# shichaoy/cube_slam

Hardware: NVIDIA H100
Metric: scored cuboid proposals/s (higher is better)
Workload: dtype f64

## Files before the change

### cube_slam_b200/csrc/cs_lsd.cu

```cuda
#include <cuda_runtime.h>
#include <float.h>
#include <math.h>
#include <stdint.h>

#include <algorithm>
#include <cmath>
#include <cstring>
#include <vector>

#include "cs_internal.h"
#include "cs_nfa.cuh"
#include "cs_tma.cuh"

#define LSD_PI 3.1415926535897932384626433832795
#define LSD_NOTDEF (-1024.0)
#define LSD_DEG2RAD (LSD_PI / 180)
#define LSD_3_2_PI ((3 * LSD_PI) / 2)
#define LSD_2PI (2 * LSD_PI)
#define LSD_LN10 2.30258509299404568402
#define LSD_NBINS 1024
#define LSD_CHUNK_ROWS 8
#define LSD_SCALE 0.8

#define LSD_CAND_CAP 2048
#define LSD_SEQ_SCAP 2048
#define LSD_SEQ_SMEM (LSD_SEQ_SCAP * 4 + 96 * 8)
#define LSD_HDR 8

namespace {

struct LsdGeom {
    int64_t img_off;
    int32_t w, h, stride, channels;
    int32_t W, H;
    int32_t min_reg_size, tile0;
    double LOG_NT;
    int64_t px_off;
    int64_t bit_off;
    int64_t arena_off;
    int32_t tiles_x, pad_;
};

__constant__ double c_gauss7[7] = {0x1.763496d347532p-13, 0x1.f1e23259cfdc1p-7, 0x1.bfd7fac1bd5a8p-3, 0x1.10562a79786afp-1,
                                   0x1.bfd7fac1bd5a8p-3, 0x1.f1e23259cfdc1p-7, 0x1.763496d347532p-13};

__device__ __forceinline__ int reflect101(int p, int n)
{
    if (n == 1) return 0;
    while (p < 0 || p >= n) p = (p < 0) ? -p : 2 * n - 2 - p;
    return p;
}

__device__ __forceinline__ float fast_atan2(float y, float x)
{
    const float p1 = 0.9997878412794807f * (float)(180 / LSD_PI);
    const float p3 = -0.3258083974640975f * (float)(180 / LSD_PI);
    const float p5 = 0.1555786518463281f * (float)(180 / LSD_PI);
    const float p7 = -0.04432655554792128f * (float)(180 / LSD_PI);
    const float ax = fabsf(x), ay = fabsf(y);
    float a, c, c2;
    if (ax >= ay) {
        c = ay / (ax + (float)DBL_EPSILON);
        c2 = c * c;
        a = (((p7 * c2 + p5) * c2 + p3) * c2 + p1) * c;
    } else {
        c = ax / (ay + (float)DBL_EPSILON);
        c2 = c * c;
        a = 90.f - (((p7 * c2 + p5) * c2 + p3) * c2 + p1) * c;
    }
    if (x < 0) a = 180.f - a;
    if (y < 0) a = 360.f - a;
    return a;
}

__device__ __forceinline__ void lsd_resize_col(int dx, int sw, double inv_scale, int &sx, float &fx, bool &single)
{
    fx = (float)((dx + 0.5) * inv_scale - 0.5);
    sx = (int)floorf(fx);
    fx -= sx;
    single = false;
    if (sx < 0) {
        fx = 0;
        sx = 0;
    }
    if (sx + 1 >= sw) {
        single = true;
        if (sx >= sw - 1) {
            fx = 0;
            sx = sw - 1;
        }
    }
}
__device__ __forceinline__ void lsd_resize_row(int dy, int sh, double inv_scale, int &y0, int &y1, float &fy)
{
    fy = (float)((dy + 0.5) * inv_scale - 0.5);
    const int sy = (int)floorf(fy);
    fy -= sy;
    y0 = (sy >= 0) ? (sy < sh ? sy : sh - 1) : 0;
    y1 = (sy + 1 >= 0) ? (sy + 1 < sh ? sy + 1 : sh - 1) : 0;
}

#define LSF_TW 32
#define LSF_TH 16
#define LSF_BW 44
#define LSF_BH 24
#define LSF_GW (LSF_BW + 6)
#define LSF_GH (LSF_BH + 6)
#define LSF_BOXW 176
#define LSF_P_BYTES (LSF_GH * LSF_BW * 8)
static_assert(LSF_GH * LSF_BOXW <= LSF_P_BYTES && (LSF_TH + 1) * (LSF_TW + 1) * 8 <= LSF_P_BYTES, "front-end shared-memory aliasing");
template <bool kTma, bool kDebug, bool kMixed>
__global__ void __launch_bounds__(256) k_lsd_front(const __grid_constant__ CUtensorMap tmap, const uint8_t *__restrict__ img, int w, int h, int stride,
                                                   int channels, int W, int H, double inv_scale, double threshold, double *__restrict__ modgrad,
                                                   float *__restrict__ angf, uint4 *__restrict__ pix, uint32_t *__restrict__ defb,
                                                   double *__restrict__ scaled, int32_t *__restrict__ err_flag, const LsdGeom *__restrict__ geom,
                                                   int n_geom)
{
    static_assert(!(kMixed && (kTma || kDebug)), "a mixed batch has no tensor map and no debug form");
    __shared__ __align__(128) unsigned char s_p[LSF_P_BYTES];
    __shared__ double s_b[LSF_BH][LSF_BW];
    __shared__ uint8_t s_g[LSF_GH][LSF_GW];
    __shared__ __align__(8) unsigned long long s_bar;
    double(*s_h)[LSF_BW] = reinterpret_cast<double(*)[LSF_BW]>(s_p);
    double(*s_sc)[LSF_TW + 1] = reinterpret_cast<double(*)[LSF_TW + 1]>(s_p);
    int f = blockIdx.z, X0 = blockIdx.x * LSF_TW, Y0 = blockIdx.y * LSF_TH;
// ... 85 lines not shown
        double s = c_gauss7[3] * s_h[r + 3][c];
#pragma unroll
        for (int k = 1; k <= 3; k++) s += c_gauss7[3 + k] * (s_h[r + 3 + k][c] + s_h[r + 3 - k][c]);
        s_b[r][c] = s;
    }
    __syncthreads();
    for (int i = tid; i < (LSF_TH + 1) * (LSF_TW + 1); i += 256) {
        const int r = i / (LSF_TW + 1), c = i - r * (LSF_TW + 1);
        if (Y0 + r > yl || X0 + c > xl) continue;
        int sx, y0, y1;
        float fx, fy;
        bool single;
        lsd_resize_col(X0 + c, w, inv_scale, sx, fx, single);
        lsd_resize_row(Y0 + r, h, inv_scale, y0, y1, fy);
        const double *S0 = s_b[y0 - by0], *S1 = s_b[y1 - by0];
        const int cx = sx - bx0;
        const float a0 = 1.f - fx, a1 = fx, b0 = 1.f - fy, b1 = fy;
        double r0, r1;
        if (!single) {
            r0 = S0[cx] * a0 + S0[cx + 1] * a1;
            r1 = S1[cx] * a0 + S1[cx + 1] * a1;
        } else {
            r0 = S0[cx] * 1.0;
            r1 = S1[cx] * 1.0;
        }
        s_sc[r][c] = r0 * b0 + r1 * b1;
    }
    __syncthreads();
    const int WW = (W + 31) >> 5;
    for (int i = tid; i < LSF_TH * LSF_TW; i += 256) {
        const int r = i / LSF_TW, c = i - r * LSF_TW;
        const int x = X0 + c, y = Y0 + r;
        float deg = -1.f;
        if (x < W && y < H) {
            const size_t p = kMixed ? (size_t)y * W + x : ((size_t)f * H + y) * W + x;
            double norm = 0;
            if (x < W - 1 && y < H - 1) {
                const double DA = s_sc[r + 1][c + 1] - s_sc[r][c];
                const double BC = s_sc[r][c + 1] - s_sc[r + 1][c];
                const double gx = DA + BC, gy = DA - BC;
                norm = sqrt((gx * gx + gy * gy) / 4);
                if (!kDebug && !(norm <= threshold)) deg = fast_atan2((float)gx, (float)(-gy));
            }
            if (kDebug) {
                scaled[p] = s_sc[r][c];
                modgrad[p] = norm;
            } else {
                angf[p] = deg;
                uint4 rec = make_uint4(__float_as_uint(deg), 0u, 0u, 0u);
                if (deg >= 0.f) {
                    modgrad[p] = norm;
                    const double ang = (double)deg * LSD_DEG2RAD;
                    const double af = (double)(float)ang;
                    rec.y = __float_as_uint((float)cos(af));
                    rec.z = __float_as_uint((float)sin(af));
                }
                pix[p] = rec;
            }
        }
        if (!kDebug) {
            const uint32_t bits = __ballot_sync(0xffffffffu, deg >= 0.f);
            if (c == 0 && y < H) defb[(kMixed ? (size_t)y : (size_t)f * H + y) * WW + (X0 >> 5)] = bits;
        }
    }
}

__device__ unsigned long long g_lsd_prof[16];
#define LSD_PROF_T0() const long long prof_t0__ = kProf ? clock64() : 0ll
#define LSD_PROF_ADD(slot)                                                                         \
    do {                                                                                           \
        if (kProf && (threadIdx.x & 31) == 0) atomicAdd(&g_lsd_prof[slot], (unsigned long long)(clock64() - prof_t0__)); \
    } while (0)
#define LSD_PROF_COUNT(slot, v)                                                    \
    do {                                                                           \
        if (kProf && (threadIdx.x & 31) == 0) atomicAdd(&g_lsd_prof[slot], (unsigned long long)(v)); \
    } while (0)
#define LSD_PROF_RECT_SIZE(n) LSD_PROF_COUNT(15, (n) <= 32 ? 1ull : (n) <= 64 ? 1ull << 21 : 1ull << 42)

extern __shared__ __align__(8) int s_seq[];
__device__ __forceinline__ double *lsd_stage() { return reinterpret_cast<double *>(s_seq + LSD_SEQ_SCAP); }

struct LsdFrame {
    int W, H;
    uint4 *pix;
    const float *angf;
    const double *modgrad;
    double LOG_NT;
    uint32_t *ubits;
    int WW;
    __device__ __forceinline__ uint32_t *used_at(int y, int x, uint32_t &bit) const
    {
        bit = 1u << (x & 31);
        return ubits + y * WW + (x >> 5);
    }
    struct LsdSpan *span;
    const double *lgam;
    unsigned long long wmagic;
    __device__ __forceinline__ int row_of(int addr) const { return (int)(((unsigned long long)(unsigned)addr * wmagic) >> 40); }
};

struct LsdReg {
    int *g;
    int cap;
    __device__ __forceinline__ int get(int i) const { return i < LSD_SEQ_SCAP ? s_seq[i] : g[i]; }
    __device__ __forceinline__ void put(int i, int v) const
    {
        if (i < LSD_SEQ_SCAP)
            s_seq[i] = v;
        else
            g[i] = v;
    }
};

__device__ __forceinline__ void lsd_prefetch_l2(const void *p) { asm volatile("prefetch.global.L2 [%0];" ::"l"(p)); }

struct LsdRect {
    double x1, y1, x2, y2, width, x, y, theta, dx, dy, prec, p;
};

__device__ __forceinline__ double lsd_dist_sq(double x1, double y1, double x2, double y2) { return (x2 - x1) * (x2 - x1) + (y2 - y1) * (y2 - y1); }
__device__ __forceinline__ double lsd_dist(double x1, double y1, double x2, double y2) { return sqrt(lsd_dist_sq(x1, y1, x2, y2)); }
__device__ __forceinline__ double lsd_angle_diff_signed(double a, double b)
{
    double diff = a - b;
    while (diff <= -LSD_PI) diff += LSD_2PI;
    while (diff > LSD_PI) diff -= LSD_2PI;
    return diff;
}
__device__ __forceinline__ bool lsd_double_equal(double a, double b)
{
    if (a == b) return true;
    const double abs_diff = fabs(a - b);
    const double aa = fabs(a), bb = fabs(b);
    double abs_max = (aa > bb) ? aa : bb;
    if (abs_max < DBL_MIN) abs_max = DBL_MIN;
    return (abs_diff / abs_max) <= (100.0 * DBL_EPSILON);
}
__device__ __forceinline__ bool lsd_aligned_deg(float deg, double theta, double prec)
{
    if (deg < 0.f) return false;
    {
        float nf = fabsf((float)theta - deg * 0.017453292f);
        if (nf > 4.712389f) nf = fabsf(nf - 6.2831855f);
        const float pf = (float)prec;
        if (nf < pf - 2e-4f) return true;
        if (nf > pf + 2e-4f) return false;
    }
    const double a = (double)deg * LSD_DEG2RAD;
    double n_theta = theta - a;
    if (n_theta < 0) n_theta = -n_theta;
    if (n_theta > LSD_3_2_PI) {
        n_theta -= LSD_2PI;
        if (n_theta < 0) n_theta = -n_theta;
    }
    return n_theta <= prec;
}

__device__ __noinline__ double lsd_log_gamma(double x)
{
    if (x > 15.0) return 0.918938533204673 + (x - 0.5) * log(x) - x + 0.5 * x * log(x * sinh(1 / x) + 1 / (810.0 * pow(x, 6.0)));
    const double q[7] = {75122.6331530, 80916.6278952, 36308.2951477, 8687.24529705, 1168.92649479, 83.8676043424, 2.50662827511};
    double a = (x + 0.5) * log(x + 5.5) - (x + 5.5);
    double b = 0;
    for (int n = 0; n < 7; ++n) {
        a -= log(x + (double)n);
        b += q[n] * pow(x, (double)n);
    }
    return a + log(b);
}

__device__ __noinline__ double lsd_nfa(int n, int k, double p, double LOG_NT)
{
    if (n == 0 || k == 0) return -LOG_NT;
    if (n == k) return -LOG_NT - (double)n * log10(p);
    const double p_term = p / (1 - p);
    const double log1term = ((double)n + 1) - lsd_log_gamma((double)k + 1) - lsd_log_gamma((double)(n - k) + 1) + (double)k * log(p) + (double)(n - k) * log(1.0 - p);
    double term = exp(log1term);
    if (lsd_double_equal(term, 0)) {
        if (k > n * p) return -log1term / LSD_LN10 - LOG_NT;
        return -LOG_NT;
    }
    double bin_tail = term;
    const double tolerance = 0.1;
    for (int i = k + 1; i <= n; ++i) {
        const double bin_term = (double)(n - i + 1) / (double)i;
        const double mult_term = bin_term * p_term;
        term *= mult_term;
        bin_tail += term;
        if (bin_term < 1) {
            const double err = term * ((1 - pow(mult_term, (double)(n - i + 1))) / (1 - mult_term) - 1);
            if (err < tolerance * fabs(-log10(bin_tail) - LOG_NT) * bin_tail) break;
        }
    }
    return -log10(bin_tail) - LOG_NT;
}

__device__ void lsd_region_grow(const LsdFrame &F, const LsdReg &R, int base, int s_addr, int &reg_size, double &reg_angle, double prec)
{
    const unsigned FULL = 0xffffffffu;
    const int lane = threadIdx.x & 31;
    float reg_deg = F.angf[s_addr];
    reg_angle = (double)reg_deg * LSD_DEG2RAD;
    float sumdx = (float)cos(reg_angle);
    float sumdy = (float)sin(reg_angle);
    __syncwarp();
    if (lane == 0) {
        const int sy = F.row_of(s_addr);
        uint32_t bit;
        uint32_t *w = F.used_at(sy, s_addr - sy * F.W, bit);
        atomicOr(w, bit);
        R.put(base, s_addr);
    }
    reg_size = 1;
    __syncwarp();
    const int grp = lane / 9, kk = lane - grp * 9;
    const int ky = kk / 3 - 1, kx = kk - (kk / 3) * 3 - 1;
    const float precf = (float)prec;
    const unsigned lt_mask = (1u << lane) - 1u;
    for (int i = 0; i < reg_size;) {
        const int navail = min(3, reg_size - i);
        bool cand = false;
        int c_addr = -1;
        float deg = -1.f, csx = 0.f, csy = 0.f;
        if (grp < navail) {
            const int pa = R.get(base + i + grp);
            const int py = F.row_of(pa), px = pa - py * F.W;
            const int yy = py + ky, xx = px + kx;
            if (yy >= 0 && yy < F.H && xx >= 0 && xx < F.W) {
                c_addr = yy * F.W + xx;
                uint32_t ubit;
                const uint32_t *uw_p = F.used_at(yy, xx, ubit);
                const uint4 r = __ldg(F.pix + c_addr);
                const uint32_t uw = __ldcg(uw_p);
                deg = __uint_as_float(r.x);
                if (deg >= 0.f && !(uw & ubit)) {
                    cand = true;
                    csx = __uint_as_float(r.y);
                    csy = __uint_as_float(r.z);
                }
            }
        }
        unsigned maybe = __ballot_sync(FULL, cand);
        if (maybe) {
            float nf = fabsf(reg_deg * 0.017453292f - deg * 0.017453292f);
            if (nf > 4.712389f) nf = fabsf(nf - 6.2831855f);
            const float inv_l = rsqrtf(sumdx * sumdx + sumdy * sumdy) * 1.001f;
            const float per_add = (precf + 0.201f) * inv_l;
            unsigned sure = 0u;
            float D = (float)__popc(maybe) * per_add + 0.0022f;
            if (D <= 0.2f && precf + D < 1.5f) {
                const unsigned m1 = __ballot_sync(FULL, cand && nf < precf + D);
                D = (float)__popc(m1) * per_add + 0.0022f;
                sure = __ballot_sync(FULL, cand && nf < precf - D);
                maybe = __ballot_sync(FULL, cand && nf < precf + D);
            }
            unsigned accepted = 0u;
            bool stale = false;
            while (maybe) {
                const int fl = __ffs(maybe) - 1;
                maybe &= ~(1u << fl);
                if (!((sure >> fl) & 1u)) {
                    if (stale) {
                        reg_deg = fast_atan2(sumdy, sumdx);
                        stale = false;
                    }
                    const bool ok = lsd_aligned_deg(deg, (double)reg_deg * LSD_DEG2RAD, prec);
                    if (!((__ballot_sync(FULL, ok) >> fl) & 1u)) continue;
                }
                const int addrf = __shfl_sync(FULL, c_addr, fl);
                sumdx += __shfl_sync(FULL, csx, fl);
                sumdy += __shfl_sync(FULL, csy, fl);
                stale = true;
                accepted |= 1u << fl;
                maybe &= ~__ballot_sync(FULL, c_addr == addrf);
            }
            if (accepted) {
                if ((accepted >> lane) & 1u) {
                    R.put(base + reg_size + __popc(accepted & lt_mask), c_addr);
                    const int cy = F.row_of(c_addr);
                    uint32_t ubit;
                    uint32_t *uw_p = F.used_at(cy, c_addr - cy * F.W, ubit);
                    atomicOr(uw_p, ubit);
                    const uint4 *q = F.pix + c_addr - 1;
                    if (c_addr >= F.W + 1) lsd_prefetch_l2(q - F.W);
                    lsd_prefetch_l2(q);
                    if (c_addr + F.W + 1 < F.W * F.H) lsd_prefetch_l2(q + F.W);
                }
                reg_size += __popc(accepted);
                if (stale) reg_deg = fast_atan2(sumdy, sumdx);
                __syncwarp();
            }
        }
        i += navail;
    }
    reg_angle = (double)reg_deg * LSD_DEG2RAD;
}

__device__ void lsd_region2rect(const LsdFrame &F, const LsdReg &R, int base, int reg_size, double reg_angle, double prec, double p, LsdRect &rec)
{
    const int lane = threadIdx.x & 31;
    double *st = lsd_stage();
    double x = 0, y = 0, sum = 0;
    for (int i0 = 0; i0 < reg_size; i0 += 32) {
        const int n = min(32, reg_size - i0);
        __syncwarp();
        if (lane < n) {
            const int addr = R.get(base + i0 + lane);
            const double weight = F.modgrad[addr];
            const int ry = F.row_of(addr), rx = addr - ry * F.W;
            st[lane] = (double)rx * weight;
            st[32 + lane] = (double)ry * weight;
            st[64 + lane] = weight;
        }
        __syncwarp();
        for (int j = 0; j < n; j++) {
            x += st[j];
            y += st[32 + j];
            sum += st[64 + j];
        }
    }
    x /= sum;
    y /= sum;
    double Ixx = 0.0, Iyy = 0.0, Ixy = 0.0;
    for (int i0 = 0; i0 < reg_size; i0 += 32) {
        const int n = min(32, reg_size - i0);
        __syncwarp();
        if (lane < n) {
            const int addr = R.get(base + i0 + lane);
            const double weight = F.modgrad[addr];
            const int ry = F.row_of(addr), rx = addr - ry * F.W;
            const double ddx = (double)rx - x, ddy = (double)ry - y;
            st[lane] = ddy * ddy * weight;
            st[32 + lane] = ddx * ddx * weight;
            st[64 + lane] = ddx * ddy * weight;
        }
        __syncwarp();
        for (int j = 0; j < n; j++) {
            Ixx += st[j];
            Iyy += st[32 + j];
            Ixy -= st[64 + j];
        }
    }
    const double lambda = 0.5 * (Ixx + Iyy - sqrt((Ixx - Iyy) * (Ixx - Iyy) + 4.0 * Ixy * Ixy));
    double theta = (fabs(Ixx) > fabs(Iyy)) ? (double)fast_atan2((float)(lambda - Ixx), (float)Ixy) : (double)fast_atan2((float)Ixy, (float)(lambda - Iyy));
    theta *= LSD_DEG2RAD;
    if (fabs(lsd_angle_diff_signed(theta, reg_angle)) > prec) theta += LSD_PI;
    const double dx = cos(theta), dy = sin(theta);
    double l_min = 0, l_max = 0, w_min = 0, w_max = 0;
    for (int i = lane; i < reg_size; i += 32) {
        const int addr = R.get(base + i);
        const int ry = F.row_of(addr), rx = addr - ry * F.W;
        const double regdx = (double)rx - x, regdy = (double)ry - y;
        const double l = regdx * dx + regdy * dy;
        const double w = -regdx * dy + regdy * dx;
        l_max = fmax(l_max, l);
        l_min = fmin(l_min, l);
        w_max = fmax(w_max, w);
        w_min = fmin(w_min, w);
    }
#pragma unroll
    for (int o = 16; o > 0; o >>= 1) {
        l_max = fmax(l_max, __shfl_xor_sync(0xffffffffu, l_max, o));
        l_min = fmin(l_min, __shfl_xor_sync(0xffffffffu, l_min, o));
        w_max = fmax(w_max, __shfl_xor_sync(0xffffffffu, w_max, o));
        w_min = fmin(w_min, __shfl_xor_sync(0xffffffffu, w_min, o));
    }
    rec.x1 = x + l_min * dx;
    rec.y1 = y + l_min * dy;
    rec.x2 = x + l_max * dx;
    rec.y2 = y + l_max * dy;
    rec.width = w_max - w_min;
    rec.x = x;
    rec.y = y;
    rec.theta = theta;
    rec.dx = dx;
    rec.dy = dy;
    rec.prec = prec;
    rec.p = p;
    if (rec.width < 1.0) rec.width = 1.0;
}

__device__ __noinline__ void lsd_region2rect_cold(const LsdFrame &F, const LsdReg &R, int base, int reg_size, double reg_angle, double prec, double p, LsdRect &rec);

template <bool kProf>
__device__ __noinline__ int lsd_reduce_region_radius(const LsdFrame &F, const LsdReg &R, int base, int &reg_size, double reg_angle, double prec, double p,
                                        LsdRect &rec, double density, double density_th)
{
    const unsigned FULL = 0xffffffffu;
    const int lane = threadIdx.x & 31;
    const unsigned lt_mask = (1u << lane) - 1u, gt_mask = ~((2u << lane) - 1u);
    int *st = reinterpret_cast<int *>(lsd_stage());
    const int a0 = R.get(base);
    const double xc = (double)(a0 - F.row_of(a0) * F.W), yc = (double)F.row_of(a0);
    const double radSq1 = lsd_dist_sq(xc, yc, rec.x1, rec.y1), radSq2 = lsd_dist_sq(xc, yc, rec.x2, rec.y2);
    double radSq = radSq1 > radSq2 ? radSq1 : radSq2;
    auto outside = [&](int addr) {
        const int ay = F.row_of(addr), ax = addr - ay * F.W;
        return lsd_dist_sq(xc, yc, (double)ax, (double)ay) > radSq;
    };
    while (density < density_th) {
        radSq *= 0.75 * 0.75;
        const int rs = reg_size;
        int K = 0;
        for (int i0 = 0; i0 < rs; i0 += 32) {
            bool out = false;
            if (i0 + lane < rs) {
                const int addr = R.get(base + i0 + lane);
                out = outside(addr);
                if (out) {
                    const int ay = F.row_of(addr);
                    uint32_t bit;
                    uint32_t *w = F.used_at(ay, addr - ay * F.W, bit);
                    atomicAnd(w, ~bit);
                }
            }
            K += __popc(__ballot_sync(FULL, i0 + lane < rs && !out));
        }
        int hc = -32, dc = (((rs - 1) >> 5) + 1) << 5, dval = 0;
        unsigned hm = 0u, dm = 0u;
        for (;;) {
            while (hm == 0u && hc + 32 < K) {
                hc += 32;
                hm = __ballot_sync(FULL, hc + lane < K && outside(R.get(base + hc + lane)));
            }
            if (hm == 0u) break;
            while (dm == 0u) {
                dc -= 32;
                const int i = dc + lane;
                dval = i < rs ? R.get(base + i) : 0;
                dm = __ballot_sync(FULL, i >= K && i < rs && !outside(dval));
            }
            const int t = min(__popc(hm), __popc(dm));
            const bool give = ((dm >> lane) & 1u) && __popc(dm & gt_mask) < t;
            const bool take = ((hm >> lane) & 1u) && __popc(hm & lt_mask) < t;
            __syncwarp();
            if (give) st[__popc(dm & gt_mask)] = dval;
            __syncwarp();
            if (take) R.put(base + hc + lane, st[__popc(hm & lt_mask)]);
            hm &= ~__ballot_sync(FULL, take);
            dm &= ~__ballot_sync(FULL, give);
        }
        reg_size = K;
        __syncwarp();
        LSD_PROF_COUNT(14, 1);
        if (reg_size < 2) return 3;
        LSD_PROF_RECT_SIZE(reg_size);
        lsd_region2rect_cold(F, R, base, reg_size, reg_angle, prec, p, rec);
        density = (double)reg_size / (lsd_dist(rec.x1, rec.y1, rec.x2, rec.y2) * rec.width);
    }
    return 0;
}

struct LsdSpan {
    int mx, ly, ry, y0, y1;
    int fl, sl, fr, sr;
};

__device__ void lsd_span_setup(const LsdFrame &F, const LsdRect &rec, LsdSpan &P)
{
    const double half_width = rec.width / 2.0;
    const double dyhw = rec.dy * half_width, dxhw = rec.dx * half_width;
    int ox[4], oy[4];
    ox[0] = (int)(rec.x1 - dyhw);
    oy[0] = (int)(rec.y1 + dxhw);
    ox[1] = (int)(rec.x2 - dyhw);
    oy[1] = (int)(rec.y2 + dxhw);
    ox[2] = (int)(rec.x2 + dyhw);
    oy[2] = (int)(rec.y2 - dxhw);
    ox[3] = (int)(rec.x1 + dyhw);
    oy[3] = (int)(rec.y1 - dxhw);
#pragma unroll
    for (int i = 1; i < 4; i++) {
        const int vx = ox[i], vy = oy[i];
        int j = i - 1;
        while (j >= 0 && ((vx == ox[j]) ? (vy < oy[j]) : (vx < ox[j]))) {
            ox[j + 1] = ox[j];
            oy[j + 1] = oy[j];
            j--;
        }
        ox[j + 1] = vx;
        oy[j + 1] = vy;
    }
    int imin = 0, imax = 0;
    for (int i = 1; i < 4; ++i) {
        if (oy[imin] > oy[i]) imin = i;
        if (oy[imax] < oy[i]) imax = i;
    }
    unsigned taken = 1u << imin;
    int ileft = -1;
    for (int i = 0; i < 4; ++i)
        if (!((taken >> i) & 1u)) {
            if (ileft < 0)
                ileft = i;
            else if (ox[ileft] > ox[i])
                ileft = i;
        }
    taken |= 1u << ileft;
    int iright = -1;
    for (int i = 0; i < 4; ++i)
        if (!((taken >> i) & 1u)) {
            if (iright < 0)
                iright = i;
            else if (ox[iright] < ox[i])
// ... 10 lines not shown
        }
    const int mx = ox[imin], my = oy[imin], lx = ox[ileft], ly = oy[ileft], rx = ox[iright], ry = oy[iright], tx = ox[itail];
    P.mx = mx;
    P.ly = ly;
    P.ry = ry;
    P.fl = (my != ly) ? (mx - lx) / (my - ly) : 0;
    P.sl = (ly != tx) ? (lx - tx) / (ly - tx) : 0;
    P.fr = (my != ry) ? (mx - rx) / (my - ry) : 0;
    P.sr = (ry != tx) ? (rx - tx) / (ry - tx) : 0;
    P.y0 = max(my, 0);
    P.y1 = min(oy[imax], F.H - 1);
}

__device__ __forceinline__ void lsd_span_row(const LsdSpan &P, int y, int W, int &lo, int &hi)
{
    const long long n_l2 = (long long)max(0, y - max(P.ly, P.y0)), n_l1 = (long long)(y - P.y0) - n_l2;
    const long long n_r2 = (long long)max(0, y - max(P.ry, P.y0)), n_r1 = (long long)(y - P.y0) - n_r2;
    const long long left_x = (long long)P.mx + n_l1 * (long long)P.fl + n_l2 * (long long)P.sl;
    const long long right_x = (long long)P.mx + n_r1 * (long long)P.fr + n_r2 * (long long)P.sr;
    lo = (int)(left_x > 0 ? left_x : 0);
    hi = (int)(right_x < (long long)(W - 1) ? right_x : (long long)(W - 1));
}

__device__ void lsd_rect_count(const LsdFrame &F, const LsdRect &rec, int &total_pts, int &alg_pts)
{
    const int lane = threadIdx.x & 31;
    LsdSpan P;
    lsd_span_setup(F, rec, P);
    int tot = 0, alg = 0;
    const int n_rows = P.y1 - P.y0 + 1;
    int G = 1;
    while (G < 32 && n_rows * G * 2 <= 32) G <<= 1;
    const int rows_per_step = 32 / G, sub = lane & (G - 1), rsel = lane / G;
    for (int yb = P.y0; yb <= P.y1; yb += rows_per_step) {
        const int y = yb + rsel;
        if (y > P.y1) continue;
        int lo, hi;
        lsd_span_row(P, y, F.W, lo, hi);
        if (hi >= lo) {
            if (sub == 0) tot += hi - lo + 1;
            const float *row = F.angf + (size_t)y * F.W;
            for (int x = lo + sub; x <= hi; x += G) alg += lsd_aligned_deg(row[x], rec.theta, rec.prec) ? 1 : 0;
        }
    }
#pragma unroll
    for (int o = 16; o > 0; o >>= 1) {
        tot += __shfl_xor_sync(0xffffffffu, tot, o);
        alg += __shfl_xor_sync(0xffffffffu, alg, o);
    }
    total_pts = tot;
    alg_pts = alg;
}

__device__ void lsd_rect_count_multi(const LsdFrame &F, const LsdRect *r, int n, bool same_geom, int *tot, int *alg)
{
    const unsigned FULL = 0xffffffffu;
    const int lane = threadIdx.x & 31;
    LsdSpan *sp = F.span;
    const int n_geom = same_geom ? 1 : n;
    __syncwarp();
    if (lane < n_geom) lsd_span_setup(F, r[lane], sp[lane]);
    __syncwarp();
    int y_min = sp[0].y0, y_max = sp[0].y1;
    for (int t = 1; t < n_geom; t++) {
        y_min = min(y_min, sp[t].y0);
        y_max = max(y_max, sp[t].y1);
    }
    const double theta = r[0].theta;
    const float thetaf = (float)theta;
    float pf[5];
#pragma unroll
    for (int t = 0; t < 5; t++) pf[t] = (float)r[t < n ? t : 0].prec;
    int c_tot[5] = {0, 0, 0, 0, 0}, c_alg[5] = {0, 0, 0, 0, 0};
    const int n_rows = y_max - y_min + 1;
    int G = 1;
    while (G < 32 && n_rows * G * 2 <= 32) G <<= 1;
    const int rows_per_step = 32 / G, sub = lane & (G - 1), rsel = lane / G;
    for (int yb = y_min; yb <= y_max; yb += rows_per_step) {
        const int y = yb + rsel;
        if (y > y_max) continue;
        int lo[5], hi[5];
        int x_lo = 0x7fffffff, x_hi = -1;
#pragma unroll
        for (int t = 0; t < 5; t++) {
            lo[t] = 1;
            hi[t] = 0;
            if (t < n_geom && y >= sp[t].y0 && y <= sp[t].y1) {
                lsd_span_row(sp[t], y, F.W, lo[t], hi[t]);
                if (hi[t] >= lo[t]) {
                    x_lo = min(x_lo, lo[t]);
                    x_hi = max(x_hi, hi[t]);
                    if (sub == 0) c_tot[t] += hi[t] - lo[t] + 1;
                }
            }
        }
        if (x_hi < 0) continue;
        const float *row = F.angf + (size_t)y * F.W;
        for (int x = x_lo + sub; x <= x_hi; x += G) {
            const float deg = row[x];
            if (deg < 0.f) continue;
            float nf = fabsf(thetaf - deg * 0.017453292f);
            if (nf > 4.712389f) nf = fabsf(nf - 6.2831855f);
            if (same_geom) {
#pragma unroll
                for (int t = 0; t < 5; t++)
                    if (t < n) {
                        bool a = nf < pf[t] - 2e-4f;
                        if (!a && !(nf > pf[t] + 2e-4f)) a = lsd_aligned_deg(deg, theta, r[t].prec);
                        c_alg[t] += a ? 1 : 0;
                    }
            } else {
                bool a = nf < pf[0] - 2e-4f;
                if (!a && !(nf > pf[0] + 2e-4f)) a = lsd_aligned_deg(deg, theta, r[0].prec);
                if (a) {
#pragma unroll
                    for (int t = 0; t < 5; t++) c_alg[t] += (x >= lo[t] && x <= hi[t]) ? 1 : 0;
                }
            }
        }
    }
    if (same_geom) {
#pragma unroll
        for (int t = 1; t < 5; t++) c_tot[t] = c_tot[0];
    }
#pragma unroll
    for (int t = 0; t < 5; t++) {
#pragma unroll
        for (int o = 16; o > 0; o >>= 1) {
            c_tot[t] += __shfl_xor_sync(FULL, c_tot[t], o);
            c_alg[t] += __shfl_xor_sync(FULL, c_alg[t], o);
        }
        if (t < n) {
            tot[t] = c_tot[t];
            alg[t] = c_alg[t];
        }
    }
}

__device__ __noinline__ void lsd_region2rect_cold(const LsdFrame &F, const LsdReg &R, int base, int reg_size, double reg_angle, double prec, double p, LsdRect &rec)
{
    lsd_region2rect(F, R, base, reg_size, reg_angle, prec, p, rec);
}

template <bool kProf>
__device__ void lsd_grow_candidate(const LsdFrame &F, const LsdReg &R, int s_addr, int min_reg_size, double prec, double p, int &n_all,
                                  int &has_rect, LsdRect &rec)
{
    const double DENSITY_TH = 0.7;
    const int lane = threadIdx.x & 31;
    int base = 0, reg_size = 0, seed = s_addr;
    double reg_angle = 0, tau = prec;
    has_rect = 0;
    n_all = 0;
    for (int pass = 0; pass < 2; pass++) {
        {
            LSD_PROF_T0();
            lsd_region_grow(F, R, base, seed, reg_size, reg_angle, tau);
            LSD_PROF_ADD(pass == 0 ? 0 : 2);
        }
        if (kProf && pass == 0 && lane == 0) {
            atomicAdd(&g_lsd_prof[5], 1ull);
            atomicAdd(&g_lsd_prof[7], (unsigned long long)reg_size);
        }
        n_all = base + reg_size;
        if (reg_size < (pass == 0 ? min_reg_size : 2)) return;
        if (pass == 0) LSD_PROF_COUNT(12, 1);
        LSD_PROF_RECT_SIZE(reg_size);
        {
            LSD_PROF_T0();
            lsd_region2rect(F, R, base, reg_size, reg_angle, prec, p, rec);
            LSD_PROF_ADD(1);
        }
        double density;
        {
            LSD_PROF_T0();
            density = (double)reg_size / (lsd_dist(rec.x1, rec.y1, rec.x2, rec.y2) * rec.width);
            has_rect = density >= DENSITY_TH;
            LSD_PROF_ADD(10);
        }
        if (has_rect) return;
        if (pass == 1) {
            LSD_PROF_T0();
            if (lsd_reduce_region_radius<kProf>(F, R, base, reg_size, reg_angle, prec, p, rec, density, DENSITY_TH) == 0) has_rect = 1;
            LSD_PROF_ADD(11);
            return;
        }
        LSD_PROF_COUNT(13, 1);
        LSD_PROF_T0();
        const int a0 = R.get(base);
        const double xc = (double)(a0 - F.row_of(a0) * F.W), yc = (double)F.row_of(a0);
        const double ang_c = (double)F.angf[a0] * LSD_DEG2RAD;
        double sum = 0, s_sum = 0;
        int n = 0;
        for (int i0 = 0; i0 < reg_size; i0 += 32) {
            const int m = min(32, reg_size - i0);
            bool near = false;
            __syncwarp();
            if (lane < m) {
                const int addr = R.get(base + i0 + lane);
                const int ry = F.row_of(addr), rx = addr - ry * F.W;
                if (lsd_dist(xc, yc, (double)rx, (double)ry) < rec.width) {
                    near = true;
                    const double ang_d = lsd_angle_diff_signed((double)F.angf[addr] * LSD_DEG2RAD, ang_c);
                    lsd_stage()[lane] = ang_d;
                    lsd_stage()[32 + lane] = ang_d * ang_d;
                }
            }
            __syncwarp();
            unsigned todo = __ballot_sync(0xffffffffu, near);
            n += __popc(todo);
            while (todo) {
                const int j = __ffs(todo) - 1;
                todo &= todo - 1;
                sum += lsd_stage()[j];
                s_sum += lsd_stage()[32 + j];
            }
        }
        for (int i = lane; i < reg_size; i += 32) {
            const int addr = R.get(base + i);
            const int ay = F.row_of(addr);
            uint32_t bit;
            uint32_t *w = F.used_at(ay, addr - ay * F.W, bit);
            atomicAnd(w, ~bit);
        }
        __syncwarp();
        const double mean_angle = sum / (double)n;
        tau = 2.0 * sqrt((s_sum - 2.0 * mean_angle * sum) / (double)n + mean_angle * mean_angle);
        seed = a0;
        base += reg_size;
        LSD_PROF_ADD(2);
    }
}

__device__ __forceinline__ bool lsd_keyline_filter(const float *raw, int img_w, int img_h, float line_length_thres, float *o)
{
    const float pre_boundary_thre = 10;
    float e[4] = {raw[0], raw[1], raw[2], raw[3]};
    if (e[0] < 0) e[0] = 0;
    if (e[0] >= img_w) e[0] = (float)img_w - 1.0f;
    if (e[2] < 0) e[2] = 0;
    if (e[2] >= img_w) e[2] = (float)img_w - 1.0f;
    if (e[1] < 0) e[1] = 0;
    if (e[1] >= img_h) e[1] = (float)img_h - 1.0f;
    if (e[3] < 0) e[3] = 0;
    if (e[3] >= img_h) e[3] = (float)img_h - 1.0f;
    const float sx = e[0], sy = e[1], ex = e[2], ey = e[3];
    if (((sx < pre_boundary_thre) && (ex < pre_boundary_thre)) || ((sx > img_w - pre_boundary_thre) && (ex > img_w - pre_boundary_thre)) ||
        ((sy < pre_boundary_thre) && (ey < pre_boundary_thre)) || ((sy > img_h - pre_boundary_thre) && (ey > img_h - pre_boundary_thre)))
        return false;
    const double ddx = (double)(e[0] - e[2]), ddy = (double)(e[1] - e[3]);
    const float line_length = (float)sqrt(ddx * ddx + ddy * ddy);
    if (!(line_length > line_length_thres)) return false;
    o[0] = sx;
    o[1] = sy;
// ... 9 lines not shown
    const double *modgrad;
    int32_t *arena;
    int arena_cap;
    double LOG_NT;
    int min_reg_size;
    double prec, p, scale;
    float line_length_thres;
    float *raw;
    int32_t *n_raw;
    float *out;
    int32_t *n_out;
    int cap;
    LsdRect *cand;
    int32_t *n_cand;
    int cand_cap;
    int32_t *cand_line;
    struct LsdCandState *cand_state;
    int32_t *err;
    const double *lgam;
    uint32_t *ubits;
    const uint32_t *defb;
    const LsdGeom *geom;
};

template <bool kProf, bool kMixed>
__global__ void __launch_bounds__(32, 21) k_lsd_grow_seq(LsdGrowArgs A)
{
    const int f = blockIdx.x, lane = threadIdx.x;
    LsdGeom G = {};
    if constexpr (kMixed) G = A.geom[f];
    const int fW = kMixed ? G.W : A.W, fH = kMixed ? G.H : A.H;
    const size_t npx = (size_t)fW * fH;
    const size_t px0 = kMixed ? (size_t)G.px_off : f * npx;
    LsdFrame F;
    LSD_PROF_T0();
    F.W = fW;
    F.H = fH;
    F.pix = A.pix + px0;
    F.angf = A.angf + px0;
    F.modgrad = A.modgrad + px0;
    F.LOG_NT = kMixed ? G.LOG_NT : A.LOG_NT;
    const int WW = (fW + 31) >> 5, n_words = WW * fH;
    const size_t w0f = kMixed ? (size_t)G.bit_off : (size_t)f * n_words;
    F.ubits = A.ubits + w0f;
    F.WW = WW;
    F.span = nullptr;
    F.lgam = A.lgam;
    F.wmagic = ((1ull << 40) + (unsigned long long)fW - 1) / (unsigned long long)fW;
    for (int i = lane; i < n_words; i += 32) F.ubits[i] = 0u;
    __syncwarp();
    LsdReg R;
    R.g = A.arena  +
          (kMixed ? (size_t)G.arena_off : (size_t)f * A.arena_cap);
    R.cap = A.arena_cap;
    const int min_reg_size = kMixed ? G.min_reg_size : A.min_reg_size;
    int n_cand = 0;
    const long long scan_t0 = kProf ? clock64() : 0ll;
    long long in_cand = 0, handoff_t0 = 0;
    const uint32_t *defb = A.defb + w0f;
    uint32_t d_next = lane < n_words ? __ldg(defb + lane) : 0u, u_next = 0u;
    for (int w0 = 0; w0 < n_words; w0 += 32) {
        const int wi = w0 + lane;
        const uint32_t d = d_next;
        uint32_t u = u_next;
        d_next = wi + 32 < n_words ? __ldg(defb + wi + 32) : 0u;
        u_next = wi + 32 < n_words ? __ldcg(F.ubits + wi + 32) : 0u;
        const int wy = wi / WW, w_addr = wy * fW + ((wi - wy * WW) << 5);
        uint32_t s = d & ~u;
        for (;;) {
            const unsigned nz = __ballot_sync(0xffffffffu, s != 0u);
            if (kProf && handoff_t0) {
                if (lane == 0) atomicAdd(&g_lsd_prof[9], (unsigned long long)(clock64() - handoff_t0));
                handoff_t0 = 0;
            }
            if (!nz) break;
            const int j = __ffs(nz) - 1;
            const int b = __ffs(__shfl_sync(0xffffffffu, s, j)) - 1;
            const int s_addr = __shfl_sync(0xffffffffu, w_addr, j) + b;
            int n_all = 0, has_rect = 0;
            LsdRect rec;
            const long long c0 = kProf ? clock64() : 0ll;
            lsd_grow_candidate<kProf>(F, R, s_addr, min_reg_size, A.prec, A.p, n_all, has_rect, rec);
            if (kProf) {
                in_cand += clock64() - c0;
                if (lane == 0) {
                    atomicAdd(&g_lsd_prof[4], 1ull);
                    if (n_all > LSD_SEQ_SCAP) atomicAdd(&g_lsd_prof[8], 1ull);
                }
            }
            if (kProf) handoff_t0 = clock64();
            __syncwarp();
            u = wi < n_words ? __ldcg(F.ubits + wi) : 0u;
            u_next = wi + 32 < n_words ? __ldcg(F.ubits + wi + 32) : 0u;
            s = d & ~u & (lane > j ? 0xffffffffu : lane == j ? 0xfffffffeu << b : 0u);
            if (!has_rect) continue;
            const long long st0 = kProf ? clock64() : 0ll;
            if (lane == 0 && n_cand < A.cand_cap) A.cand[(size_t)f * A.cand_cap + n_cand] = rec;
            n_cand++;
            if (kProf) {
                const long long dt = clock64() - st0;
                if (lane == 0) atomicAdd(&g_lsd_prof[10], (unsigned long long)dt);
                handoff_t0 += dt;
            }
        }
    }
    if (kProf && lane == 0) atomicAdd(&g_lsd_prof[3], (unsigned long long)(clock64() - scan_t0 - in_cand));
    if (lane == 0) {
        A.n_cand[f] = n_cand;
        if (n_cand > A.cand_cap) {
            atomicOr(A.err, 4);
            atomicMax(A.err + 1, n_cand);
            A.err[2] = A.cand_cap;
        }
    }
    LSD_PROF_ADD(6);
}

#define LSD_VAL_CTAS 64

struct LsdCandState {
    double log_nfa;
    int32_t status;
    int32_t n;
    int32_t tot[5], alg[5];
};

__device__ int lsd_improve_variants(const LsdRect &rec, int round, LsdRect *cand)
{
    const double delta = 0.5, delta_2 = delta / 2.0;
    LsdRect r = rec;
    if (round == 0) {
        cand[0] = r;
        return 1;
    }
    if (round == 1) {
        for (int n = 0; n < 5; ++n) {
            r.p /= 2;
            r.prec = r.p * LSD_PI;
            cand[n] = r;
        }
        return 5;
    }
    const int phase = round - 2;
    int m = 0;
    for (int n = 0; n < 5; ++n)
        if ((r.width - delta) >= 0.5) {
            if (phase == 0)
                r.width -= delta;
            else if (phase == 1) {
                r.x1 += -r.dy * delta_2;
                r.y1 += r.dx * delta_2;
                r.x2 += -r.dy * delta_2;
                r.y2 += r.dx * delta_2;
                r.width -= delta;
            } else if (phase == 2) {
                r.x1 -= -r.dy * delta_2;
                r.y1 -= r.dx * delta_2;
                r.x2 -= -r.dy * delta_2;
                r.y2 -= r.dx * delta_2;
                r.width -= delta;
            } else {
                r.p /= 2;
                r.prec = r.p * LSD_PI;
            }
            cand[m++] = r;
        }
    return m;
}

template <bool kMixed>
__global__ void __launch_bounds__(128, 5) k_lsd_val_count(LsdGrowArgs A, int round)
{
    const int f = kMixed ? (int)(blockIdx.x / LSD_VAL_CTAS) : (int)blockIdx.y, lane = threadIdx.x & 31;
    const int bx = kMixed ? (int)(blockIdx.x % LSD_VAL_CTAS) : (int)blockIdx.x, gx = kMixed ? LSD_VAL_CTAS : (int)gridDim.x;
    LsdFrame F;
    if constexpr (kMixed) {
        const LsdGeom &G = A.geom[f];
        F.W = G.W;
        F.H = G.H;
        F.angf = A.angf + G.px_off;
        F.LOG_NT = G.LOG_NT;
    } else {
        const size_t npx = (size_t)A.W * A.H;
        F.W = A.W;
        F.H = A.H;
        F.angf = A.angf + f * npx;
        F.LOG_NT = A.LOG_NT;
    }
    F.pix = nullptr;
    F.modgrad = nullptr;
    F.ubits = nullptr;
    __shared__ LsdSpan s_span[4][5];
    F.span = s_span[threadIdx.x >> 5];
    F.lgam = A.lgam;
    F.wmagic = 0;
    const int n = min(A.n_cand[f], A.cand_cap);
    const int wpb = blockDim.x >> 5;
    for (int c = bx * wpb + (threadIdx.x >> 5); c < n; c += gx * wpb) {
        LsdCandState *S = A.cand_state + (size_t)f * A.cand_cap + c;
        if (round > 0 && S->status != 0) continue;
        const LsdRect rec = A.cand[(size_t)f * A.cand_cap + c];
        LsdRect cv[5];
        const int m = lsd_improve_variants(rec, round, cv);
        int tot[5] = {0, 0, 0, 0, 0}, alg[5] = {0, 0, 0, 0, 0};
        if (m == 1)
            lsd_rect_count(F, cv[0], tot[0], alg[0]);
        else if (m > 1)
            lsd_rect_count_multi(F, cv, m, round == 1 || round == 5, tot, alg);
        if (lane == 0) {
            S->n = m;
            for (int t = 0; t < 5; t++) {
                S->tot[t] = tot[t];
                S->alg[t] = alg[t];
            }
        }
    }
}

template <bool kMixed>
__global__ void __launch_bounds__(128, 5) k_lsd_val_nfa(LsdGrowArgs A, int round)
{
    const int f = kMixed ? (int)(blockIdx.x / LSD_VAL_CTAS) : (int)blockIdx.y, lane = threadIdx.x & 31;
    const int bx = kMixed ? (int)(blockIdx.x % LSD_VAL_CTAS) : (int)blockIdx.x, gx = kMixed ? LSD_VAL_CTAS : (int)gridDim.x;
    const double LOG_NT = kMixed ? A.geom[f].LOG_NT : A.LOG_NT;
    const int n = min(A.n_cand[f], A.cand_cap);
    const int wpb = blockDim.x >> 5;
    for (int c = bx * wpb + (threadIdx.x >> 5); c < n; c += gx * wpb) {
        LsdCandState *S = A.cand_state + (size_t)f * A.cand_cap + c;
        if (round > 0 && S->status != 0) continue;
        LsdRect rec = A.cand[(size_t)f * A.cand_cap + c];
        LsdRect cv[5];
        const int m = lsd_improve_variants(rec, round, cv);
        double log_nfa = round == 0 ? 0.0 : S->log_nfa;
        bool changed = false;
        for (int t = 0; t < m; t++) {
            const double v = cs_nfa_warp(A.lgam, S->tot[t], S->alg[t], cv[t].p, LOG_NT, true);
            if (round == 0 || v > log_nfa) {
                log_nfa = v;
                rec = cv[t];
                changed = round > 0;
            }
        }
        const bool done = round == 5 || log_nfa > 0.0;
        __syncwarp();
        if (lane == 0) {
            if (done) {
                int32_t *o = A.cand_line + ((size_t)f * A.cand_cap + c) * 5;
                const bool ok = log_nfa > 0.0;
                o[0] = ok ? 1 : 0;
                o[1] = __float_as_int((float)((rec.x1 + 0.5) / A.scale));
                o[2] = __float_as_int((float)((rec.y1 + 0.5) / A.scale));
                o[3] = __float_as_int((float)((rec.x2 + 0.5) / A.scale));
                o[4] = __float_as_int((float)((rec.y2 + 0.5) / A.scale));
                S->status = 1;
            } else {
                if (changed) A.cand[(size_t)f * A.cand_cap + c] = rec;
                S->log_nfa = log_nfa;
                S->status = 0;
            }
        }
    }
}

#define LSD_LAUNCHES_PER_RUN 15

template <bool kMixed>
__global__ void __launch_bounds__(256) k_lsd_emit(LsdGrowArgs A)
{
    __shared__ int s_warp_cnt[8], s_base_raw, s_base_out;
    const int f = blockIdx.x, tid = threadIdx.x, lane = tid & 31, wid = tid >> 5;
    const unsigned FULL = 0xffffffffu;
    const int n = min(A.n_cand[f], A.cand_cap);
    float *raw = A.raw + (size_t)f * A.cap * 4;
    float *out = A.out + (size_t)f * A.cap * 4;
    if (tid == 0) {
        s_base_raw = 0;
        s_base_out = 0;
    }
    __syncthreads();
    for (int b = 0; b < n; b += 256) {
        const int i = b + tid;
        bool has = false, kept = false;
        float ln[4], fo[4];
        if (i < n) {
            const int32_t *o = A.cand_line + ((size_t)f * A.cand_cap + i) * 5;
            if (o[0]) {
                has = true;
                for (int k = 0; k < 4; k++) ln[k] = __int_as_float(o[1 + k]);
                kept = lsd_keyline_filter(ln, kMixed ? A.geom[f].w : A.img_w, kMixed ? A.geom[f].h : A.img_h, A.line_length_thres, fo);
            }
        }
        const unsigned mh = __ballot_sync(FULL, has), mk = __ballot_sync(FULL, kept);
        if (lane == 0) s_warp_cnt[wid] = __popc(mh) | (__popc(mk) << 16);
        __syncthreads();
        int pre_r = s_base_raw, pre_o = s_base_out;
// ... 651 lines not shown
```

Baseline: 9.171 million.

## Cut register pressure in LSD kernels via shared rect staging and on-demand variants

Stops passing LsdRect by reference through the grow, reduce and rect paths and stores the rectangle in shared staging memory instead. Replaces the five-entry LsdRect variant arrays with variants recomputed on demand per lane or per index, keeping only precisions in shared memory. Adds range assumptions to cos and sin so the compiler can drop the slow argument-reduction path. The aim is to lower register and local-memory use and shrink the noinline call interfaces. The cost is repeated arithmetic for variants and extra shared-memory traffic.

```diff
diff --git a/cube_slam_b200/csrc/cs_lsd.cu b/cube_slam_b200/csrc/cs_lsd.cu
--- a/cube_slam_b200/csrc/cs_lsd.cu
+++ b/cube_slam_b200/csrc/cs_lsd.cu
@@ -71,6 +71,17 @@
     if (x < 0) a = 180.f - a;
     if (y < 0) a = 360.f - a;
     return a;
+}
+
+__device__ __forceinline__ double lsd_cos(double a)
+{
+    __builtin_assume(!(fabs(a) >= 2147483648.0));
+    return cos(a);
+}
+__device__ __forceinline__ double lsd_sin(double a)
+{
+    __builtin_assume(!(fabs(a) >= 2147483648.0));
+    return sin(a);
 }
 
 __device__ __forceinline__ void lsd_resize_col(int dx, int sw, double inv_scale, int &sx, float &fx, bool &single)
@@ -262,8 +273,8 @@
                     modgrad[p] = norm;
                     const double ang = (double)deg * LSD_DEG2RAD;
                     const double af = (double)(float)ang;
-                    rec.y = __float_as_uint((float)cos(af));
-                    rec.z = __float_as_uint((float)sin(af));
+                    rec.y = __float_as_uint((float)lsd_cos(af));
+                    rec.z = __float_as_uint((float)lsd_sin(af));
                 }
                 pix[p] = rec;
             }
@@ -311,7 +322,6 @@
 
 struct LsdReg {
     int *g;
-    int cap;
     __device__ __forceinline__ int get(int i) const { return i < LSD_SEQ_SCAP ? s_seq[i] : g[i]; }
     __device__ __forceinline__ void put(int i, int v) const
     {
@@ -327,6 +337,7 @@
 struct LsdRect {
     double x1, y1, x2, y2, width, x, y, theta, dx, dy, prec, p;
 };
+__device__ __forceinline__ LsdRect *lsd_rect() { return reinterpret_cast<LsdRect *>(lsd_stage() + 64); }
 
 __device__ __forceinline__ double lsd_dist_sq(double x1, double y1, double x2, double y2) { return (x2 - x1) * (x2 - x1) + (y2 - y1) * (y2 - y1); }
 __device__ __forceinline__ double lsd_dist(double x1, double y1, double x2, double y2) { return sqrt(lsd_dist_sq(x1, y1, x2, y2)); }
@@ -411,8 +422,8 @@
     const int lane = threadIdx.x & 31;
     float reg_deg = F.angf[s_addr];
     reg_angle = (double)reg_deg * LSD_DEG2RAD;
-    float sumdx = (float)cos(reg_angle);
-    float sumdy = (float)sin(reg_angle);
+    float sumdx = (float)lsd_cos(reg_angle);
+    float sumdy = (float)lsd_sin(reg_angle);
     __syncwarp();
     if (lane == 0) {
         const int sy = F.row_of(s_addr);
@@ -506,7 +517,7 @@
     reg_angle = (double)reg_deg * LSD_DEG2RAD;
 }
 
-__device__ void lsd_region2rect(const LsdFrame &F, const LsdReg &R, int base, int reg_size, double reg_angle, double prec, double p, LsdRect &rec)
+__device__ void lsd_region2rect(const LsdFrame &F, const LsdReg &R, int base, int reg_size, double reg_angle, double prec, double p)
 {
     const int lane = threadIdx.x & 31;
     double *st = lsd_stage();
@@ -555,7 +566,7 @@
     double theta = (fabs(Ixx) > fabs(Iyy)) ? (double)fast_atan2((float)(lambda - Ixx), (float)Ixy) : (double)fast_atan2((float)Ixy, (float)(lambda - Iyy));
     theta *= LSD_DEG2RAD;
     if (fabs(lsd_angle_diff_signed(theta, reg_angle)) > prec) theta += LSD_PI;
-    const double dx = cos(theta), dy = sin(theta);
+    const double dx = lsd_cos(theta), dy = lsd_sin(theta);
     double l_min = 0, l_max = 0, w_min = 0, w_max = 0;
     for (int i = lane; i < reg_size; i += 32) {
         const int addr = R.get(base + i);
@@ -575,6 +586,7 @@
         w_max = fmax(w_max, __shfl_xor_sync(0xffffffffu, w_max, o));
         w_min = fmin(w_min, __shfl_xor_sync(0xffffffffu, w_min, o));
     }
+    LsdRect rec;
     rec.x1 = x + l_min * dx;
     rec.y1 = y + l_min * dy;
     rec.x2 = x + l_max * dx;
@@ -588,21 +600,38 @@
     rec.prec = prec;
     rec.p = p;
     if (rec.width < 1.0) rec.width = 1.0;
-}
-
-__device__ __noinline__ void lsd_region2rect_cold(const LsdFrame &F, const LsdReg &R, int base, int reg_size, double reg_angle, double prec, double p, LsdRect &rec);
+    __syncwarp();
+    if (lane == 0) *lsd_rect() = rec;
+    __syncwarp();
+}
+
+__device__ __forceinline__ LsdFrame lsd_frame_of(int W, unsigned long long wmagic, uint32_t *ubits, int WW, const double *modgrad)
+{
+    LsdFrame F = {};
+    F.W = W;
+    F.wmagic = wmagic;
+    F.ubits = ubits;
+    F.WW = WW;
+    F.modgrad = modgrad;
+    return F;
+}
+__device__ __noinline__ void lsd_region2rect_cold(int W, unsigned long long wmagic, const double *modgrad, int *g, int base, int reg_size, double reg_angle,
+                                                  double prec, double p);
 
 template <bool kProf>
-__device__ __noinline__ int lsd_reduce_region_radius(const LsdFrame &F, const LsdReg &R, int base, int &reg_size, double reg_angle, double prec, double p,
-                                        LsdRect &rec, double density, double density_th)
+__device__ __noinline__ bool lsd_reduce_region_radius(int W, unsigned long long wmagic, uint32_t *ubits, int WW, const double *modgrad, int *g, int base,
+                                                      int reg_size, double reg_angle, double prec, double p, double density, double density_th)
 {
     const unsigned FULL = 0xffffffffu;
     const int lane = threadIdx.x & 31;
     const unsigned lt_mask = (1u << lane) - 1u, gt_mask = ~((2u << lane) - 1u);
+    const LsdFrame F = lsd_frame_of(W, wmagic, ubits, WW, modgrad);
+    const LsdReg R = {g};
     int *st = reinterpret_cast<int *>(lsd_stage());
     const int a0 = R.get(base);
     const double xc = (double)(a0 - F.row_of(a0) * F.W), yc = (double)F.row_of(a0);
-    const double radSq1 = lsd_dist_sq(xc, yc, rec.x1, rec.y1), radSq2 = lsd_dist_sq(xc, yc, rec.x2, rec.y2);
+    const LsdRect *rec = lsd_rect();
+    const double radSq1 = lsd_dist_sq(xc, yc, rec->x1, rec->y1), radSq2 = lsd_dist_sq(xc, yc, rec->x2, rec->y2);
     double radSq = radSq1 > radSq2 ? radSq1 : radSq2;
     auto outside = [&](int addr) {
         const int ay = F.row_of(addr), ax = addr - ay * F.W;
@@ -653,12 +682,50 @@
         reg_size = K;
         __syncwarp();
         LSD_PROF_COUNT(14, 1);
-        if (reg_size < 2) return 3;
+        if (reg_size < 2) return false;
         LSD_PROF_RECT_SIZE(reg_size);
-        lsd_region2rect_cold(F, R, base, reg_size, reg_angle, prec, p, rec);
-        density = (double)reg_size / (lsd_dist(rec.x1, rec.y1, rec.x2, rec.y2) * rec.width);
-    }
-    return 0;
+        lsd_region2rect_cold(W, wmagic, modgrad, g, base, reg_size, reg_angle, prec, p);
+        density = (double)reg_size / (lsd_dist(rec->x1, rec->y1, rec->x2, rec->y2) * rec->width);
+    }
+    return true;
+}
+
+__device__ __forceinline__ bool lsd_improve_step(LsdRect &r, int round)
+{
+    const double delta = 0.5, delta_2 = delta / 2.0;
+    if (round >= 2 && !((r.width - delta) >= 0.5)) return false;
+    if (round == 1 || round == 5) {
+        r.p /= 2;
+        r.prec = r.p * LSD_PI;
+    } else if (round == 2)
+        r.width -= delta;
+    else if (round == 3) {
+        r.x1 += -r.dy * delta_2;
+        r.y1 += r.dx * delta_2;
+        r.x2 += -r.dy * delta_2;
+        r.y2 += r.dx * delta_2;
+        r.width -= delta;
+    } else {
+        r.x1 -= -r.dy * delta_2;
+        r.y1 -= r.dx * delta_2;
+        r.x2 -= -r.dy * delta_2;
+        r.y2 -= r.dx * delta_2;
+        r.width -= delta;
+    }
+    return true;
+}
+__device__ __forceinline__ int lsd_improve_count(LsdRect r, int round)
+{
+    if (round == 0) return 1;
+    int m = 0;
+    while (m < 5 && lsd_improve_step(r, round)) m++;
+    return m;
+}
+__device__ __forceinline__ LsdRect lsd_improve_variant(LsdRect r, int round, int t)
+{
+    if (round > 0)
+        for (int k = 0; k <= t; k++) lsd_improve_step(r, round);
+    return r;
 }
 
 struct LsdSpan {
@@ -775,25 +842,29 @@
     alg_pts = alg;
 }
 
-__device__ void lsd_rect_count_multi(const LsdFrame &F, const LsdRect *r, int n, bool same_geom, int *tot, int *alg)
+__device__ void lsd_rect_count_multi(const LsdFrame &F, const LsdRect &rec, int round, int n, bool same_geom, double *prec, int *tot, int *alg)
 {
     const unsigned FULL = 0xffffffffu;
     const int lane = threadIdx.x & 31;
     LsdSpan *sp = F.span;
     const int n_geom = same_geom ? 1 : n;
     __syncwarp();
-    if (lane < n_geom) lsd_span_setup(F, r[lane], sp[lane]);
+    if (lane < n) {
+        const LsdRect v = lsd_improve_variant(rec, round, lane);
+        prec[lane] = v.prec;
+        if (lane < n_geom) lsd_span_setup(F, v, sp[lane]);
+    }
     __syncwarp();
     int y_min = sp[0].y0, y_max = sp[0].y1;
     for (int t = 1; t < n_geom; t++) {
         y_min = min(y_min, sp[t].y0);
         y_max = max(y_max, sp[t].y1);
     }
-    const double theta = r[0].theta;
+    const double theta = rec.theta;
     const float thetaf = (float)theta;
     float pf[5];
 #pragma unroll
-    for (int t = 0; t < 5; t++) pf[t] = (float)r[t < n ? t : 0].prec;
+    for (int t = 0; t < 5; t++) pf[t] = (float)prec[t < n ? t : 0];
     int c_tot[5] = {0, 0, 0, 0, 0}, c_alg[5] = {0, 0, 0, 0, 0};
     const int n_rows = y_max - y_min + 1;
     int G = 1;
@@ -829,12 +900,12 @@
                 for (int t = 0; t < 5; t++)
                     if (t < n) {
                         bool a = nf < pf[t] - 2e-4f;
-                        if (!a && !(nf > pf[t] + 2e-4f)) a = lsd_aligned_deg(deg, theta, r[t].prec);
+                        if (!a && !(nf > pf[t] + 2e-4f)) a = lsd_aligned_deg(deg, theta, prec[t]);
                         c_alg[t] += a ? 1 : 0;
                     }
             } else {
                 bool a = nf < pf[0] - 2e-4f;
-                if (!a && !(nf > pf[0] + 2e-4f)) a = lsd_aligned_deg(deg, theta, r[0].prec);
+                if (!a && !(nf > pf[0] + 2e-4f)) a = lsd_aligned_deg(deg, theta, prec[0]);
                 if (a) {
 #pragma unroll
                     for (int t = 0; t < 5; t++) c_alg[t] += (x >= lo[t] && x <= hi[t]) ? 1 : 0;
@@ -860,14 +931,16 @@
     }
 }
 
-__device__ __noinline__ void lsd_region2rect_cold(const LsdFrame &F, const LsdReg &R, int base, int reg_size, double reg_angle, double prec, double p, LsdRect &rec)
-{
-    lsd_region2rect(F, R, base, reg_size, reg_angle, prec, p, rec);
+__device__ __noinline__ void lsd_region2rect_cold(int W, unsigned long long wmagic, const double *modgrad, int *g, int base, int reg_size, double reg_angle,
+                                                  double prec, double p)
+{
+    const LsdReg R = {g};
+    lsd_region2rect(lsd_frame_of(W, wmagic, nullptr, 0, modgrad), R, base, reg_size, reg_angle, prec, p);
 }
 
 template <bool kProf>
 __device__ void lsd_grow_candidate(const LsdFrame &F, const LsdReg &R, int s_addr, int min_reg_size, double prec, double p, int &n_all,
-                                  int &has_rect, LsdRect &rec)
+                                  int &has_rect)
 {
     const double DENSITY_TH = 0.7;
     const int lane = threadIdx.x & 31;
@@ -891,20 +964,22 @@
         LSD_PROF_RECT_SIZE(reg_size);
         {
             LSD_PROF_T0();
-            lsd_region2rect(F, R, base, reg_size, reg_angle, prec, p, rec);
+            lsd_region2rect(F, R, base, reg_size, reg_angle, prec, p);
             LSD_PROF_ADD(1);
         }
         double density;
         {
             LSD_PROF_T0();
-            density = (double)reg_size / (lsd_dist(rec.x1, rec.y1, rec.x2, rec.y2) * rec.width);
+            const LsdRect *rec = lsd_rect();
+            density = (double)reg_size / (lsd_dist(rec->x1, rec->y1, rec->x2, rec->y2) * rec->width);
             has_rect = density >= DENSITY_TH;
             LSD_PROF_ADD(10);
         }
         if (has_rect) return;
         if (pass == 1) {
             LSD_PROF_T0();
-            if (lsd_reduce_region_radius<kProf>(F, R, base, reg_size, reg_angle, prec, p, rec, density, DENSITY_TH) == 0) has_rect = 1;
+            has_rect = lsd_reduce_region_radius<kProf>(F.W, F.wmagic, F.ubits, F.WW, F.modgrad, R.g, base, reg_size, reg_angle, prec, p, density,
+                                                       DENSITY_TH);
             LSD_PROF_ADD(11);
             return;
         }
@@ -922,7 +997,7 @@
             if (lane < m) {
                 const int addr = R.get(base + i0 + lane);
                 const int ry = F.row_of(addr), rx = addr - ry * F.W;
-                if (lsd_dist(xc, yc, (double)rx, (double)ry) < rec.width) {
+                if (lsd_dist(xc, yc, (double)rx, (double)ry) < lsd_rect()->width) {
                     near = true;
                     const double ang_d = lsd_angle_diff_signed((double)F.angf[addr] * LSD_DEG2RAD, ang_c);
                     lsd_stage()[lane] = ang_d;
@@ -1038,7 +1113,6 @@
     LsdReg R;
     R.g = A.arena  +
           (kMixed ? (size_t)G.arena_off : (size_t)f * A.arena_cap);
-    R.cap = A.arena_cap;
     const int min_reg_size = kMixed ? G.min_reg_size : A.min_reg_size;
     int n_cand = 0;
     const long long scan_t0 = kProf ? clock64() : 0ll;
@@ -1064,9 +1138,8 @@
             const int b = __ffs(__shfl_sync(0xffffffffu, s, j)) - 1;
             const int s_addr = __shfl_sync(0xffffffffu, w_addr, j) + b;
             int n_all = 0, has_rect = 0;
-            LsdRect rec;
             const long long c0 = kProf ? clock64() : 0ll;
-            lsd_grow_candidate<kProf>(F, R, s_addr, min_reg_size, A.prec, A.p, n_all, has_rect, rec);
+            lsd_grow_candidate<kProf>(F, R, s_addr, min_reg_size, A.prec, A.p, n_all, has_rect);
             if (kProf) {
                 in_cand += clock64() - c0;
                 if (lane == 0) {
@@ -1081,7 +1154,7 @@
             s = d & ~u & (lane > j ? 0xffffffffu : lane == j ? 0xfffffffeu << b : 0u);
             if (!has_rect) continue;
             const long long st0 = kProf ? clock64() : 0ll;
-            if (lane == 0 && n_cand < A.cand_cap) A.cand[(size_t)f * A.cand_cap + n_cand] = rec;
+            if (lane == 0 && n_cand < A.cand_cap) A.cand[(size_t)f * A.cand_cap + n_cand] = *lsd_rect();
             n_cand++;
             if (kProf) {
                 const long long dt = clock64() - st0;
@@ -1110,49 +1183,6 @@
     int32_t n;
     int32_t tot[5], alg[5];
 };
-
-__device__ int lsd_improve_variants(const LsdRect &rec, int round, LsdRect *cand)
-{
-    const double delta = 0.5, delta_2 = delta / 2.0;
-    LsdRect r = rec;
-    if (round == 0) {
-        cand[0] = r;
-        return 1;
-    }
-    if (round == 1) {
-        for (int n = 0; n < 5; ++n) {
-            r.p /= 2;
-            r.prec = r.p * LSD_PI;
-            cand[n] = r;
-        }
-        return 5;
-    }
-    const int phase = round - 2;
-    int m = 0;
-    for (int n = 0; n < 5; ++n)
-        if ((r.width - delta) >= 0.5) {
-            if (phase == 0)
-                r.width -= delta;
-            else if (phase == 1) {
-                r.x1 += -r.dy * delta_2;
-                r.y1 += r.dx * delta_2;
-                r.x2 += -r.dy * delta_2;
-                r.y2 += r.dx * delta_2;
-                r.width -= delta;
-            } else if (phase == 2) {
-                r.x1 -= -r.dy * delta_2;
-                r.y1 -= r.dx * delta_2;
-                r.x2 -= -r.dy * delta_2;
-                r.y2 -= r.dx * delta_2;
-                r.width -= delta;
-            } else {
-                r.p /= 2;
-                r.prec = r.p * LSD_PI;
-            }
-            cand[m++] = r;
-        }
-    return m;
-}
 
 template <bool kMixed>
 __global__ void __launch_bounds__(128, 5) k_lsd_val_count(LsdGrowArgs A, int round)
@@ -1177,6 +1207,7 @@
     F.modgrad = nullptr;
     F.ubits = nullptr;
     __shared__ LsdSpan s_span[4][5];
+    __shared__ double s_prec[4][5];
     F.span = s_span[threadIdx.x >> 5];
     F.lgam = A.lgam;
     F.wmagic = 0;
@@ -1186,13 +1217,12 @@
         LsdCandState *S = A.cand_state + (size_t)f * A.cand_cap + c;
         if (round > 0 && S->status != 0) continue;
         const LsdRect rec = A.cand[(size_t)f * A.cand_cap + c];
-        LsdRect cv[5];
-        const int m = lsd_improve_variants(rec, round, cv);
+        const int m = lsd_improve_count(rec, round);
         int tot[5] = {0, 0, 0, 0, 0}, alg[5] = {0, 0, 0, 0, 0};
         if (m == 1)
-            lsd_rect_count(F, cv[0], tot[0], alg[0]);
+            lsd_rect_count(F, lsd_improve_variant(rec, round, 0), tot[0], alg[0]);
         else if (m > 1)
-            lsd_rect_count_multi(F, cv, m, round == 1 || round == 5, tot, alg);
+            lsd_rect_count_multi(F, rec, round, m, round == 1 || round == 5, s_prec[threadIdx.x >> 5], tot, alg);
         if (lane == 0) {
             S->n = m;
             for (int t = 0; t < 5; t++) {
@@ -1215,18 +1245,19 @@
         LsdCandState *S = A.cand_state + (size_t)f * A.cand_cap + c;
         if (round > 0 && S->status != 0) continue;
         LsdRect rec = A.cand[(size_t)f * A.cand_cap + c];
-        LsdRect cv[5];
-        const int m = lsd_improve_variants(rec, round, cv);
+        const int m = lsd_improve_count(rec, round);
         double log_nfa = round == 0 ? 0.0 : S->log_nfa;
-        bool changed = false;
+        int best = -1;
         for (int t = 0; t < m; t++) {
-            const double v = cs_nfa_warp(A.lgam, S->tot[t], S->alg[t], cv[t].p, LOG_NT, true);
+            const double p = lsd_improve_variant(rec, round, t).p;
+            const double v = cs_nfa_warp(A.lgam, S->tot[t], S->alg[t], p, LOG_NT, true);
             if (round == 0 || v > log_nfa) {
                 log_nfa = v;
-                rec = cv[t];
-                changed = round > 0;
-            }
-        }
+                best = t;
+            }
+        }
+        const bool changed = round > 0 && best >= 0;
+        if (changed) rec = lsd_improve_variant(rec, round, best);
         const bool done = round == 5 || log_nfa > 0.0;
         __syncwarp();
         if (lane == 0) {
```

Result: faster. 9.341 million, median of 6 (+1.8%).
